# tildearrow/openwebrx

Hardware: NVIDIA B200
Metric: channel-MS/s (input MS/s x clients) + waterfall FFT frames/s (higher is better)
Workload: dtype f32

## Files before the change

### openwebrx_b200/csrc/selector.cu

```cuda
#include "selector_kernels.cuh"
#include "fastconv.cuh"
#include "ingress.cuh"

#include <algorithm>
#include <chrono>
#include <cmath>
#include <complex>
#include <cstdlib>
#include <deque>
#include <map>
#include <memory>
#include <mutex>
#include <vector>

using namespace owrx;

namespace {

int filter_len(double transition)
{
    int len = (int)(4.0 / transition);
    if ((len & 1) == 0) len += 1;
    return len;
}
// ... 248 lines not shown
    float* d_fc_h = nullptr; float2* d_fc_tab = nullptr; float4* d_fc_F = nullptr; float2* d_fc_Z = nullptr;
    float fc_tab_scale = 1.0f;
    float* d_fc_scale = nullptr;
    int* d_fc_slots = nullptr; double* d_fc_rates = nullptr;
    size_t fc_blocks_cap = 0;
    std::vector<double> fc_tab_rate;
    void* d_fc_tabp = nullptr; void* d_fc_Fp = nullptr; size_t fc_blocks_cap_tc = 0;
    std::vector<double> fc_tabp_rate;
    std::vector<float> fc_taps;
};

}

struct owrx_bank {
    int device = 0, sm_count = 0;
    double input_rate = 0.0;
    cudaStream_t stream = nullptr;
    cudaEvent_t ev0 = nullptr, ev1 = nullptr;
    std::mutex mu;
    std::vector<std::unique_ptr<Chan>> chans;
    std::vector<std::unique_ptr<Group>> groups;
    int out_mask = OWRX_OUT_AUDIO;
    float2* d_iq[2] = {nullptr, nullptr};
    int iq_cur = 0;
    size_t iq_cap = 0, iq_fill = 0;
    float* h_stage = nullptr; size_t h_stage_cap = 0;
    float* d_xpose = nullptr; size_t d_xpose_cap = 0;
    struct AsyncDrainItem { int which, width; size_t n, off; std::vector<int> chans; };
    float* h_adrain = nullptr; size_t h_adrain_cap = 0;
    float* d_adrain = nullptr; size_t d_adrain_cap = 0;
    std::vector<AsyncDrainItem> adrain_items;
    bool adrain_pending = false;
    cudaEvent_t adrain_done = nullptr;
    owrx_bank_stats_t stats{};
    cudaStream_t copy_stream = nullptr, side_stream = nullptr, serial_stream = nullptr;
    std::vector<cudaEvent_t> chunk_events;
    cudaEvent_t fir_done = nullptr, ptail_done[2] = {nullptr, nullptr}, tail_done[2] = {nullptr, nullptr}, dev_done = nullptr;
    bool pipelined = false, reserve_sm = false;
    std::vector<cudaEvent_t> fir_events, drain_events;
    cudaStream_t drain_stream = nullptr;
    unsigned long long calls = 0;
    bool profile = false;
    std::vector<std::pair<cudaEvent_t, cudaEvent_t>> prof_events;
    std::vector<int> prof_tags;
    size_t prof_used = 0;
    double prof_ms[OWRX_PROF_KINDS] = {};
    uint64_t prof_launches[OWRX_PROF_KINDS] = {};
    int fir_mode = OWRX_FIR_AUTO, bp_mode = OWRX_FIR_AUTO;
    unsigned char* d_raw = nullptr; size_t raw_cap = 0;
    bool deferred = false, pending_final = false;
    cudaEvent_t carry_done = nullptr;
    int fir_form_used = 0;
    bool tail_fused = true;
    bool agc_cta = true;
    size_t last_consumed = 0;
    std::vector<std::pair<std::unique_ptr<Group>, cudaEvent_t>> graveyard;
    cudaStream_t ctl_stream = nullptr;
    unsigned long long feeds = 0;
};

namespace {

template <typename T> int dev_alloc(T** p, size_t n)
{
    *p = nullptr;
    OWRX_CUDA(cudaMalloc((void**)p, std::max<size_t>(n, 1) * sizeof(T)));
    OWRX_CUDA(cudaMemset(*p, 0, std::max<size_t>(n, 1) * sizeof(T)));
    return OWRX_OK;
}

void group_release(Group* g)
{
    cudaFree(g->d_taps); cudaFree(g->d_deemph); cudaFree(g->d_pre);
    cudaFree(g->d_rate); cudaFree(g->d_phase); cudaFree(g->d_w);
    cudaFree(g->d_bp); cudaFree(g->d_bp_en2[0]); cudaFree(g->d_bp_en2[1]); cudaFree(g->d_cfg2[0]); cudaFree(g->d_cfg2[1]);
    cudaFree(g->d_state); cudaFree(g->d_stash); cudaFree(g->d_patch[0]); cudaFree(g->d_patch[1]);
    cudaFree(g->d_bp_stage); cudaFree(g->d_bp_stage_slots);
    for (int k = 0; k < 2; k++) {
        if (g->h_bp_pin[k]) cudaFreeHost(g->h_bp_pin[k]);
        if (g->bp_pin_ev[k]) cudaEventDestroy(g->bp_pin_ev[k]);
    }
    cudaFree(g->d_bp_H); cudaFree(g->d_bp_X); cudaFree(g->d_bp_Y);
    cudaFree(g->d_partial); cudaFree(g->d_gate); cudaFree(g->d_power); cudaFree(g->d_dcmean); cudaFree(g->d_dcprev);
    cudaFree(g->d_tail_mode2[0]); cudaFree(g->d_tail_mode2[1]); cudaFree(g->d_tail); cudaFree(g->d_tail_count); cudaFree(g->d_tail_s16);
    cudaFree(g->d_tail_bytes);
    cudaFree(g->d_fc_h); cudaFree(g->d_fc_tab); cudaFree(g->d_fc_F); cudaFree(g->d_fc_Z); cudaFree(g->d_fc_slots); cudaFree(g->d_fc_rates);
    cudaFree(g->d_fc_scale);
    cudaFree(g->d_fc_tabp); cudaFree(g->d_fc_Fp);
    g->s1.release(); g->s2.release(); g->s3.release(); g->f1.release(); g->f1p.release(); g->f1b.release(); g->f2.release(); g->f3.release();
}

owrx_chan_spec_t spec_from_rates(double input_rate, double output_rate)
{
    owrx_chan_spec_t sp{};
    double orate = output_rate > input_rate ? input_rate : output_rate;
    const double d = input_rate / orate;
    sp.decimation = (int)d;
    sp.fraction = (input_rate / sp.decimation) / orate;
    sp.transition = 0.15 * (orate / input_rate);
    sp.cutoff = 0.5 * sp.decimation / (input_rate / orate);
    sp.bp_transition = 320.0 / orate;
    sp.squelch_length = std::max(1, (int)(orate / 16));
    sp.deemph_rate = (int)orate;
    return sp;
}

bool spec_equal(const owrx_chan_spec_t& a, const owrx_chan_spec_t& b)
// ... 758 lines not shown
                for (size_t o = 0; o < nv; o += kRowChunk * BP_RB) {
                    const size_t c = std::min(kRowChunk * BP_RB, nv - o);
                    fir_fwd_f_kernel<<<grid2d(S, (c + BP_RB - 1) / BP_RB), kBlock2d, 0, st>>>(src + o * S, S, (int)c, last_row - (int)o, g->d_pre,
                                                                                           g->Tpre, g->f1p.append_ptr() + o * S);
                    OWRX_LAUNCH_CHECK();
                }
                g->f1p.appended(nv);
            }
            size_t cnt = 0;
            while (true) {
                const double where = 5.0 + (double)(g->wfm_m + (long long)cnt) * g->wfm_rate;
                if ((long long)ceil(where) + 6 >= g->f1p.abs_end) break;
                cnt++;
            }
            if ((rc = g->f1b.ensure_new(cnt, st)) != OWRX_OK) return rc;
            if ((rc = g->f2.ensure_new(cnt, st)) != OWRX_OK) return rc;
            for (size_t o = 0; o < cnt; o += kRowChunk) {
                const size_t c = std::min(kRowChunk, cnt - o);
                fracdec_f_kernel<<<grid2d(S, c), kBlock2d, 0, st>>>(g->f1p.rows(), g->f1p.abs_end - (long long)g->f1p.fill, S,
                                                                    g->wfm_rate, g->wfm_m + (long long)o, (int)c, nullptr, 0,
                                                                    g->f1b.append_ptr() + o * S);
                OWRX_LAUNCH_CHECK();
            }
            if (cnt) {
                wfm_deemph_kernel<<<S / IIR_CH, IIR_TL, 0, st>>>(g->f1b.append_ptr(), S, (int)cnt, g->alpha, g->d_state,
                                                                  g->f2.append_ptr());
                OWRX_LAUNCH_CHECK();
            }
            bank->stats.kernel_launches += 2;
            g->wfm_m += (long long)cnt;
            g->f2.appended(cnt);
            n_audio = cnt;
        }
        g->last_demod += n_audio;
        g->last_audio += n_audio;
        g->pass_audio = n_audio;
    }
    return OWRX_OK;
}

int group_tail_serial(owrx_bank* bank, Group* g, cudaStream_t st)
{
    const int S = g->slots;
    const size_t n_audio = g->pass_audio;
    int rc;
    {
        if (n_audio) {
            if ((rc = g->f3.ensure_new(n_audio, st)) != OWRX_OK) return rc;
            if ((rc = prof_mark(bank, OWRX_PROF_AGC, st, true)) != OWRX_OK) return rc;
            if (g->wfm) {
                OWRX_CUDA(cudaMemcpyAsync(g->f3.append_ptr(), g->f2.rows(g->f2.fill - n_audio), n_audio * (size_t)S * sizeof(float),
                                          cudaMemcpyDeviceToDevice, st));
            } else {
                static const int agc_pad = (getenv("OWRX_AGC_PAD_KB") ? atoi(getenv("OWRX_AGC_PAD_KB")) : 160) << 10;
                const bool agc_cta = bank->agc_cta;
                static const int agcw_pad = (getenv("OWRX_AGCW_PAD_KB") ? atoi(getenv("OWRX_AGCW_PAD_KB")) : 0) << 10;
                if (agc_cta) {
                    if (agc_pad) OWRX_CUDA(cudaFuncSetAttribute(agc_kernel, cudaFuncAttributeMaxDynamicSharedMemorySize, agc_pad));
                    agc_kernel<<<S / AGC_CH, AGC_TL, agc_pad, st>>>(g->f2.rows(g->f2.fill - n_audio), S, (int)n_audio, g->d_cfg, g->d_state,
                                                               g->f3.append_ptr());
                } else {
                    if (agcw_pad) OWRX_CUDA(cudaFuncSetAttribute(agc_warp_kernel, cudaFuncAttributeMaxDynamicSharedMemorySize, agcw_pad));
                    agc_warp_kernel<<<S, 32, agcw_pad, st>>>(g->f2.rows(g->f2.fill - n_audio), S, (int)n_audio, g->d_cfg, g->d_state,
                                                           g->f3.append_ptr());
                }
                OWRX_LAUNCH_CHECK();
            }
            if ((rc = prof_mark(bank, OWRX_PROF_AGC, st, false)) != OWRX_OK) return rc;
            bank->stats.kernel_launches++;
            g->f3.appended(n_audio);
            if (g->any_tail) {
                const size_t row0 = g->last_audio - n_audio;
                if (g->last_audio > g->tail_rows_cap) return fail(OWRX_E_STATE, "audio tail scratch under-provisioned");
                audio_tail_kernel<<<(S + 31) / 32, 128, 0, st>>>(g->f3.rows(g->f3.fill - n_audio), S, (int)n_audio, g->d_tail_mode,
                                                               g->d_tail, g->d_tail_s16 + row0 * (size_t)S, g->d_tail_bytes,
                                                               g->d_tail_count, g->tail_cap);
                OWRX_LAUNCH_CHECK();
                bank->stats.kernel_launches++;
                g->tail_ran = true;
            }
        }
    }
    return OWRX_OK;
}

int group_begin_feed(owrx_bank* bank, Group* g, size_t rows, cudaStream_t st_fir, cudaStream_t st_tail, cudaStream_t st_serial, int parity)
{
    const int S = g->slots;
    int rc;
    g->cur = parity & 1;
    const size_t blocks = rows / (size_t)g->sq_len + 2;
    const size_t low = rows + (size_t)g->sq_len + 64;
    if ((rc = g->s1.roll(g->s1.hist, st_fir)) != OWRX_OK) return rc;
    if (g->has_frac && (rc = g->s2.roll(g->s2.hist, st_tail)) != OWRX_OK) return rc;
    if ((rc = g->s3.roll(g->s3.hist, st_tail)) != OWRX_OK) return rc;
    if ((rc = g->f1.roll(g->f1.hist, st_tail)) != OWRX_OK) return rc;
    if (g->wfm) { g->f1b.roll(0, st_tail); if ((rc = g->f1p.roll(g->f1p.hist, st_tail)) != OWRX_OK) return rc; }
    g->f2.roll(0, st_tail);
    g->f3.roll(0, st_tail);
    g->last_audio = g->last_demod = g->last_if = g->last_blocks = 0;
    g->dr_audio = g->dr_demod = g->dr_if = g->dr_blocks = 0;
    g->pass_audio = 0; g->feed_blocks = 0; g->tail_ran = false;
    const bool grow = g->s1.fill + rows > g->s1.cap_rows || (g->has_frac && g->s2.fill + low > g->s2.cap_rows) ||
                      g->s3.fill + low > g->s3.cap_rows || g->f1.fill + low > g->f1.cap_rows || low > g->f2.cap_rows ||
                      low > g->f3.cap_rows || (g->wfm && (low > g->f1b.cap_rows || g->f1p.fill + low > g->f1p.cap_rows)) || blocks > g->blocks_cap ||
                      (g->any_tail && low > g->tail_rows_cap);
    if (grow) {
        OWRX_CUDA(cudaDeviceSynchronize());
        if ((rc = g->s1.ensure_new(rows, st_fir)) != OWRX_OK) return rc;
        if (g->has_frac && (rc = g->s2.ensure_new(low, st_tail)) != OWRX_OK) return rc;
        if ((rc = g->s3.ensure_new(low, st_tail)) != OWRX_OK) return rc;
        if ((rc = g->f1.ensure_new(low, st_tail)) != OWRX_OK) return rc;
        if (g->wfm && (rc = g->f1b.ensure_new(low, st_tail)) != OWRX_OK) return rc;
        if (g->wfm && (rc = g->f1p.ensure_new(low, st_tail)) != OWRX_OK) return rc;
        if ((rc = g->f2.ensure_new(low, st_tail)) != OWRX_OK) return rc;
        if ((rc = g->f3.ensure_new(low, st_tail)) != OWRX_OK) return rc;
        if (blocks > g->blocks_cap) {
// ... 1056 lines not shown
```

### openwebrx_b200/csrc/selector_kernels.cuh

```cuda
#pragma once
#include "common.cuh"
#include "adpcm.cuh"

namespace owrx {

constexpr int K3_NW = 12;
constexpr int K3_CN = 2;
constexpr int K3_PP = 28;
constexpr int K3_RBMAX = 896;
constexpr int K3_CG = 32 * K3_CN;

struct K3Params {
    const float2* iq;
    long long n_lim;
    const float* taps;
    const double* ch_rate;
    const double* ch_phase;
    const float2* ch_w;
    float2* partial;
    float2* side;
    int D, nseg, nrs, RB, JB, n_blocks, n_k, slots;
};

__device__ __forceinline__ void cp_async8(void* smem_dst, const void* gsrc)
// ... 637 lines not shown
            const float4* xv = reinterpret_cast<const float4*>(&xin[buf][w][IIR_E * lane]);
            const float4 a = xv[0], b = xv[1];
            v[0] = a.x; v[1] = a.y; v[2] = a.z; v[3] = a.w; v[4] = b.x; v[5] = b.y; v[6] = b.z; v[7] = b.w;
        }
        float sl = 0.f;
#pragma unroll
        for (int e = 0; e < IIR_E; e++) sl = alpha * v[e] + om * sl;
        float B = sl;
#pragma unroll
        for (int k = 0; k < 5; k++) {
            const float prev = __shfl_up_sync(0xffffffffu, B, 1 << k);
            if (lane >= (1 << k)) B = om_pow[k] * prev + B;
        }
        float A = 1.f;
#pragma unroll
        for (int k = 0; k < 5; k++)
            if ((lane + 1) & (1 << k)) A *= om_pow[k];
        if (lane == 31) A = om_pow[5];
        const float endstate = A * y + B;
        float yin = __shfl_up_sync(0xffffffffu, endstate, 1);
        if (lane == 0) yin = y;
        float yo[IIR_E];
#pragma unroll
        for (int e = 0; e < IIR_E; e++) { yin = alpha * v[e] + om * yin; yo[e] = yin; }
        {
            float4* ov = reinterpret_cast<float4*>(&xout[w][IIR_E * lane]);
            ov[0] = make_float4(yo[0], yo[1], yo[2], yo[3]);
            ov[1] = make_float4(yo[4], yo[5], yo[6], yo[7]);
        }
        const int valid = min(IIR_TL, n - tile * IIR_TL);
        const int ll = (valid - 1) / IIR_E, le = (valid - 1) % IIR_E;
        float cand = yo[IIR_E - 1];
#pragma unroll
        for (int e = 0; e < IIR_E - 1; e++) cand = le == e ? yo[e] : cand;
        y = __shfl_sync(0xffffffffu, cand, ll);
        __syncthreads();
        const int t = tile * IIR_TL + tid;
        if (t < n) {
            float4* p = reinterpret_cast<float4*>(out + (size_t)t * slots + s0);
            p[0] = make_float4(xout[0][tid], xout[1][tid], xout[2][tid], xout[3][tid]);
            p[1] = make_float4(xout[4][tid], xout[5][tid], xout[6][tid], xout[7][tid]);
        }
        if (tile + 1 < nt) stage(buf ^ 1, lo, hi);
        __syncthreads();
    }
    if (lane == 0) st[s].iir = y;
}

constexpr int AGC_CH = 8;
constexpr int AGC_TL = 256;

constexpr int AGC_E = 4;

struct AgcWarp {
    float gain, dn, up, thr, gmax;
    int hang, hang_time;
    __device__ __forceinline__ void step_dense(float (&v)[AGC_E], int lane, float* Ud)
    {
        const unsigned full = 0xffffffffu;
        float o[AGC_E];
        int j0 = 0;
        while (true) {
            const int R = max(32 * AGC_E - j0 - hang, 0);
            float u = gain;
            Ud[3] = u;
#pragma unroll
            for (int c = 0; c < 32 * AGC_E / 4; c++) {
                if (4 * c + 4 <= R) {
                    const float a = u * up, b = a * up, cc = b * up, d = cc * up;
                    *reinterpret_cast<float4*>(&Ud[4 * c + 4]) = make_float4(a, b, cc, d);
                    u = d;
                }
            }
            for (int k = (R & ~3) + 1; k <= R; k++) {
                u *= up;
                Ud[k + 3] = u;
            }
            __syncwarp();
            float gb[AGC_E], ga[AGC_E];
            unsigned att = 0, pend = 0;
#pragma unroll
            for (int e = 0; e < AGC_E; e++) {
                const int d = AGC_E * lane + e - j0;
                const int rb = max(d - hang, 0);
                const int is_rise = d >= hang ? 1 : 0;
                const int idx = max(rb, 0);
                gb[e] = fminf(Ud[idx + 3], gmax);
                ga[e] = fminf(Ud[idx + is_rise + 3], gmax);
                const bool p = d >= 0;
                pend |= (p ? 1u : 0u) << e;
                att |= (p && fabsf(v[e]) * gb[e] > thr ? 1u : 0u) << e;
            }
            __syncwarp();
            const unsigned am = __ballot_sync(full, att != 0u);
            if (am == 0u) {
#pragma unroll
                for (int e = 0; e < AGC_E; e++)
                    if ((pend >> e) & 1u) o[e] = fminf(1.f, fmaxf(-1.f, v[e] * ga[e]));
                gain = fminf(u, gmax);
                hang = max(hang - (32 * AGC_E - j0), 0);
                break;
            }
            const int L = __ffs(am) - 1;
            const int ef = __ffs(att) - 1;
            const float gsel = ef == 0 ? gb[0] : (ef == 1 ? gb[1] : (ef == 2 ? gb[2] : gb[3]));
            const int e_first = __shfl_sync(full, ef, L);
            const float gnew = fmaxf(fminf(__shfl_sync(full, gsel, L) * dn, gmax), 0.f);
            const int jf = AGC_E * L + e_first;
#pragma unroll
            for (int e = 0; e < AGC_E; e++) {
                const int j = AGC_E * lane + e;
                if (((pend >> e) & 1u) && j < jf) o[e] = fminf(1.f, fmaxf(-1.f, v[e] * ga[e]));
                if (j == jf) o[e] = fminf(1.f, fmaxf(-1.f, v[e] * gnew));
            }
            gain = gnew;
            hang = hang_time;
            j0 = jf + 1;
            if (j0 >= 32 * AGC_E) break;
        }
#pragma unroll
        for (int e = 0; e < AGC_E; e++) v[e] = o[e];
    }

    __device__ __forceinline__ void step(float (&v)[AGC_E], int lane, volatile float* U)
    {
        const unsigned full = 0xffffffffu, lt = (1u << lane) - 1u;
        unsigned nzbits = 0;
#pragma unroll
        for (int e = 0; e < AGC_E; e++) nzbits |= (v[e] != 0.f ? 1u : 0u) << e;
        if (__all_sync(full, nzbits == 0xfu)) {
            step_dense(v, lane, const_cast<float*>(U));
            return;
        }
        float o[AGC_E];
#pragma unroll
        for (int e = 0; e < AGC_E; e++) o[e] = v[e];
        int j0 = 0;
        while (true) {
            const int sh = min(max(j0 - AGC_E * lane, 0), AGC_E);
            const unsigned act = (0xfu << sh) & 0xfu;
            const unsigned live = nzbits & act;
            unsigned m[AGC_E];
#pragma unroll
            for (int e = 0; e < AGC_E; e++) m[e] = __ballot_sync(full, (live >> e) & 1u);
            int base = 0, n_live = 0;
#pragma unroll
            for (int e = 0; e < AGC_E; e++) { base += __popc(m[e] & lt); n_live += __popc(m[e]); }
            unsigned rise = 0;
#pragma unroll
            for (int e = 0; e < AGC_E; e++) {
                const int before = base + __popc(live & ((1u << e) - 1u));
                rise |= (((live >> e) & 1u) && before >= hang ? 1u : 0u) << e;
            }
            int rbase = 0, R = 0;
#pragma unroll
            for (int e = 0; e < AGC_E; e++) {
                const unsigned r = __ballot_sync(full, (rise >> e) & 1u);
                rbase += __popc(r & lt);
                R += __popc(r);
            }
            float u = gain;
            U[0] = u;
#pragma unroll 8
            for (int k = 1; k <= R; k++) {
                u *= up;
                U[k] = u;
            }
            __syncwarp();
            float gb[AGC_E], ga[AGC_E];
            unsigned att = 0;
#pragma unroll
            for (int e = 0; e < AGC_E; e++) {
                const int rb = rbase + __popc(rise & ((1u << e) - 1u));
                gb[e] = fminf(U[rb], gmax);
                ga[e] = fminf(U[rb + ((rise >> e) & 1u)], gmax);
                att |= (((live >> e) & 1u) && fabsf(v[e]) * gb[e] > thr ? 1u : 0u) << e;
            }
            __syncwarp();
            const unsigned am = __ballot_sync(full, att != 0u);
            if (am == 0u) {
#pragma unroll
                for (int e = 0; e < AGC_E; e++)
                    if ((act >> e) & 1u) o[e] = fminf(1.f, fmaxf(-1.f, v[e] * ga[e]));
                gain = fminf(u, gmax);
                hang = max(hang - n_live, 0);
                break;
            }
            const int L = __ffs(am) - 1;
            const int ef = __ffs(att) - 1;
            const float gsel = ef == 0 ? gb[0] : (ef == 1 ? gb[1] : (ef == 2 ? gb[2] : gb[3]));
            const int e_first = __shfl_sync(full, ef, L);
            const float gnew = fmaxf(fminf(__shfl_sync(full, gsel, L) * dn, gmax), 0.f);
            const int jf = AGC_E * L + e_first;
#pragma unroll
            for (int e = 0; e < AGC_E; e++) {
                const int j = AGC_E * lane + e;
                if (((act >> e) & 1u) && j < jf) o[e] = fminf(1.f, fmaxf(-1.f, v[e] * ga[e]));
                if (j == jf) o[e] = fminf(1.f, fmaxf(-1.f, v[e] * gnew));
            }
            gain = gnew;
            hang = hang_time;
            j0 = jf + 1;
            if (j0 >= 32 * AGC_E) break;
        }
#pragma unroll
        for (int e = 0; e < AGC_E; e++) v[e] = o[e];
    }
};

__global__ void __launch_bounds__(AGC_TL)
agc_kernel(const float* __restrict__ in, int slots, int n, const ChanCfg* __restrict__ cfg, ChanState* __restrict__ st,
           float* __restrict__ out)
{
    __shared__ __align__(16) float xin[2][AGC_CH][AGC_TL];
    __shared__ __align__(16) float xout[AGC_CH][AGC_TL];
    __shared__ __align__(16) float U_all[AGC_CH][32 * AGC_E + 8];
    if (n <= 0) return;
    const int tid = threadIdx.x, lane = tid & 31, w = tid >> 5;
    const int s0 = blockIdx.x * AGC_CH, s = s0 + w;
    const ChanCfg c = cfg[s];
    const bool bypass = c.kind == OWRX_DEMOD_WFM || c.kind == OWRX_DEMOD_NONE;
    AgcWarp a{st[s].agc_gain, 1.f - c.agc_attack, 1.f + c.agc_decay, c.agc_thr, c.agc_max, st[s].agc_hang, c.agc_hang_time};
    a.gain = fmaxf(fminf(a.gain, a.gmax), 0.f);
    volatile float* U = U_all[w];
    const int nt = (n + AGC_TL - 1) / AGC_TL;
    const float4 zero4 = make_float4(0.f, 0.f, 0.f, 0.f);
    auto fetch = [&](int tile, float4& lo, float4& hi) {
        const int t = tile * AGC_TL + tid;
        if (t < n) {
            const float4* p = reinterpret_cast<const float4*>(in + (size_t)t * slots + s0);
            lo = __ldg(p); hi = __ldg(p + 1);
        } else {
            lo = zero4; hi = zero4;
        }
    };
    auto stage = [&](int buf, const float4& lo, const float4& hi) {
        xin[buf][0][tid] = lo.x; xin[buf][1][tid] = lo.y; xin[buf][2][tid] = lo.z; xin[buf][3][tid] = lo.w;
        xin[buf][4][tid] = hi.x; xin[buf][5][tid] = hi.y; xin[buf][6][tid] = hi.z; xin[buf][7][tid] = hi.w;
    };
    float4 lo, hi;
    fetch(0, lo, hi);
    stage(0, lo, hi);
    __syncthreads();
    for (int tile = 0; tile < nt; tile++) {
        const int buf = tile & 1;
        if (tile + 1 < nt) fetch(tile + 1, lo, hi);
#pragma unroll 1
        for (int k = 0; k < AGC_TL / (32 * AGC_E); k++) {
            const float4 x4 = *reinterpret_cast<const float4*>(&xin[buf][w][k * 32 * AGC_E + AGC_E * lane]);
            float v[AGC_E] = {x4.x, x4.y, x4.z, x4.w};
            if (!bypass) a.step(v, lane, U);
            *reinterpret_cast<float4*>(&xout[w][k * 32 * AGC_E + AGC_E * lane]) = make_float4(v[0], v[1], v[2], v[3]);
        }
        __syncthreads();
        const int t = tile * AGC_TL + tid;
        if (t < n) {
            float4* p = reinterpret_cast<float4*>(out + (size_t)t * slots + s0);
            p[0] = make_float4(xout[0][tid], xout[1][tid], xout[2][tid], xout[3][tid]);
            p[1] = make_float4(xout[4][tid], xout[5][tid], xout[6][tid], xout[7][tid]);
        }
        if (tile + 1 < nt) stage(buf ^ 1, lo, hi);
        __syncthreads();
    }
    if (lane == 0 && !bypass) {
        st[s].agc_gain = a.gain;
        st[s].agc_hang = a.hang;
    }
}

constexpr int AGCW_STAGES = 4;
__global__ void __launch_bounds__(32)
agc_warp_kernel(const float* __restrict__ in, int slots, int n, const ChanCfg* __restrict__ cfg, ChanState* __restrict__ st,
                float* __restrict__ out)
{
    __shared__ __align__(16) float ring[AGCW_STAGES][32 * AGC_E];
    __shared__ __align__(16) float U[32 * AGC_E + 8];
    if (n <= 0) return;
    const int lane = threadIdx.x;
    const int s = blockIdx.x;
    const ChanCfg c = cfg[s];
    const bool bypass = c.kind == OWRX_DEMOD_WFM || c.kind == OWRX_DEMOD_NONE;
    AgcWarp a{st[s].agc_gain, 1.f - c.agc_attack, 1.f + c.agc_decay, c.agc_thr, c.agc_max, st[s].agc_hang, c.agc_hang_time};
    a.gain = fmaxf(fminf(a.gain, a.gmax), 0.f);
    constexpr int SL = 32 * AGC_E;
    const int ns = (n + SL - 1) / SL;
    const float* src = in + s;
    auto issue = [&](int step) {
        if (step < ns) {
            const int i0 = step * SL + AGC_E * lane;
#pragma unroll
            for (int e = 0; e < AGC_E; e++) {
                float* dst = &ring[step % AGCW_STAGES][AGC_E * lane + e];
                if (i0 + e < n) cp_async4(dst, src + (size_t)(i0 + e) * slots);
                else *dst = 0.f;
            }
        }
        cp_async_commit();
    };
#pragma unroll
    for (int k = 0; k < AGCW_STAGES - 1; k++) issue(k);
    for (int step = 0; step < ns; step++) {
        issue(step + AGCW_STAGES - 1);
        cp_async_wait<AGCW_STAGES - 1>();
        __syncwarp();
        const float4 x4 = *reinterpret_cast<const float4*>(&ring[step % AGCW_STAGES][AGC_E * lane]);
        float v[AGC_E] = {x4.x, x4.y, x4.z, x4.w};
        if (!bypass) a.step(v, lane, U);
        const int i0 = step * SL + AGC_E * lane;
#pragma unroll
        for (int e = 0; e < AGC_E; e++)
            if (i0 + e < n) out[(size_t)(i0 + e) * slots + s] = v[e];
        __syncwarp();
    }
    if (lane == 0 && !bypass) {
        st[s].agc_gain = a.gain;
        st[s].agc_hang = a.hang;
    }
}

template <typename T>
__global__ void __launch_bounds__(256) transpose_kernel(const T* __restrict__ in, int slots, size_t n, T* __restrict__ out)
{
    __shared__ T tile[32][33];
    const int s0 = blockIdx.x * 32;
    const size_t i0 = (size_t)blockIdx.y * 32;
    for (int r = threadIdx.y; r < 32; r += 8) {
        const size_t i = i0 + r;
        const int sl = s0 + threadIdx.x;
        if (i < n && sl < slots) tile[r][threadIdx.x] = in[i * slots + sl];
    }
    __syncthreads();
    for (int r = threadIdx.y; r < 32; r += 8) {
        const int sl = s0 + r;
        const size_t i = i0 + threadIdx.x;
        if (i < n && sl < slots) out[(size_t)sl * n + i] = tile[threadIdx.x][r];
    }
}

struct TailState {
    int index, pred, since_sync, have_lo, lo;
};

constexpr int AT_R = 32;
constexpr int AT_OB = 36;
__device__ __forceinline__ void at_bar_sync(int id) { asm volatile("barrier.sync %0, 128;" ::"r"(id) : "memory"); }
__device__ __forceinline__ void at_bar_arrive(int id) { asm volatile("barrier.arrive %0, 128;" ::"r"(id) : "memory"); }

__global__ void __launch_bounds__(128)
audio_tail_kernel(const float* __restrict__ in, int slots, int n, const int* __restrict__ mode, TailState* __restrict__ ts,
                  int16_t* __restrict__ s16_out, unsigned char* __restrict__ bytes_out, int* __restrict__ count_out, int cap)
{
    __shared__ uint4 succ[IMA_TABLE_ENTRIES];
    __shared__ int qt[2][AT_R][32];
    __shared__ unsigned char obuf[2][32][AT_OB];
    __shared__ int onb[2][32];
    const int lane = threadIdx.x & 31, w = threadIdx.x >> 5;
    ima_build_table(succ, threadIdx.x, 128);
    const int s = blockIdx.x * 32 + lane;
    const bool live = s < slots;
    const int sc = live ? s : slots - 1;
    const int md = live ? mode[sc] : 0;
    if (__syncthreads_and(md == 0)) return;
    const int n_tiles = (n + AT_R - 1) / AT_R;
    constexpr int FULL = 1, EMPTY = 3;
    if (w == 0) {
// ... 137 lines not shown
```

Measured before the change: 3.549 million.

## Replace per-channel warp AGC with 512-sample tiled multi-channel AGC kernel

Replaces the one-warp-per-channel cp.async AGC kernel with a tile kernel in which each block handles 8 channels. Each warp processes 512 samples (16 per lane) per step, and loads and stores go through a shared-memory transpose using coalesced float4 accesses. AgcWarp becomes a template over elements per lane. The dense path now fills the gain ramp in chunks of 16 and stops early once the gain hits its maximum, skipping the ramp entirely when already saturated. The default switches to this new path, with dynamic shared memory padded to the device opt-in maximum to limit occupancy. The risks are more register pressure from 16 values per lane and serialized warps when attacks are frequent.

```diff
diff --git a/openwebrx_b200/csrc/selector.cu b/openwebrx_b200/csrc/selector.cu
--- a/openwebrx_b200/csrc/selector.cu
+++ b/openwebrx_b200/csrc/selector.cu
@@ -324,7 +324,7 @@
     cudaEvent_t carry_done = nullptr;
     int fir_form_used = 0;
     bool tail_fused = true;
-    bool agc_cta = true;
+    bool agc_cta = false;
     size_t last_consumed = 0;
     std::vector<std::pair<std::unique_ptr<Group>, cudaEvent_t>> graveyard;
     cudaStream_t ctl_stream = nullptr;
@@ -1189,17 +1189,26 @@
                 OWRX_CUDA(cudaMemcpyAsync(g->f3.append_ptr(), g->f2.rows(g->f2.fill - n_audio), n_audio * (size_t)S * sizeof(float),
                                           cudaMemcpyDeviceToDevice, st));
             } else {
-                static const int agc_pad = (getenv("OWRX_AGC_PAD_KB") ? atoi(getenv("OWRX_AGC_PAD_KB")) : 160) << 10;
-                const bool agc_cta = bank->agc_cta;
-                static const int agcw_pad = (getenv("OWRX_AGCW_PAD_KB") ? atoi(getenv("OWRX_AGCW_PAD_KB")) : 0) << 10;
-                if (agc_cta) {
+                static const int pad_env = getenv("OWRX_AGC_PAD_KB") ? atoi(getenv("OWRX_AGC_PAD_KB")) << 10 : -1;
+                if (bank->agc_cta) {
+                    const int agc_pad = pad_env >= 0 ? pad_env : 160 << 10;
                     if (agc_pad) OWRX_CUDA(cudaFuncSetAttribute(agc_kernel, cudaFuncAttributeMaxDynamicSharedMemorySize, agc_pad));
                     agc_kernel<<<S / AGC_CH, AGC_TL, agc_pad, st>>>(g->f2.rows(g->f2.fill - n_audio), S, (int)n_audio, g->d_cfg, g->d_state,
                                                                g->f3.append_ptr());
                 } else {
-                    if (agcw_pad) OWRX_CUDA(cudaFuncSetAttribute(agc_warp_kernel, cudaFuncAttributeMaxDynamicSharedMemorySize, agcw_pad));
-                    agc_warp_kernel<<<S, 32, agcw_pad, st>>>(g->f2.rows(g->f2.fill - n_audio), S, (int)n_audio, g->d_cfg, g->d_state,
-                                                           g->f3.append_ptr());
+                    static int full_pad = -1;
+                    if (full_pad < 0) {
+                        int dev = 0, optin = 0;
+                        cudaFuncAttributes fa{};
+                        OWRX_CUDA(cudaGetDevice(&dev));
+                        OWRX_CUDA(cudaDeviceGetAttribute(&optin, cudaDevAttrMaxSharedMemoryPerBlockOptin, dev));
+                        OWRX_CUDA(cudaFuncGetAttributes(&fa, agc_tile_kernel));
+                        full_pad = std::max(optin - (int)fa.sharedSizeBytes, 0);
+                    }
+                    const int agc_pad = pad_env >= 0 ? pad_env : full_pad;
+                    if (agc_pad) OWRX_CUDA(cudaFuncSetAttribute(agc_tile_kernel, cudaFuncAttributeMaxDynamicSharedMemorySize, agc_pad));
+                    agc_tile_kernel<<<S / AGC_CH, AGC_TL, agc_pad, st>>>(g->f2.rows(g->f2.fill - n_audio), S, (int)n_audio, g->d_cfg,
+                                                                    g->d_state, g->f3.append_ptr());
                 }
                 OWRX_LAUNCH_CHECK();
             }
diff --git a/openwebrx_b200/csrc/selector_kernels.cuh b/openwebrx_b200/csrc/selector_kernels.cuh
--- a/openwebrx_b200/csrc/selector_kernels.cuh
+++ b/openwebrx_b200/csrc/selector_kernels.cuh
@@ -713,109 +713,125 @@
 
 constexpr int AGC_E = 4;
 
+template <int E>
 struct AgcWarp {
+    static constexpr int W = 32 * E;
     float gain, dn, up, thr, gmax;
     int hang, hang_time;
-    __device__ __forceinline__ void step_dense(float (&v)[AGC_E], int lane, float* Ud)
+    __device__ __forceinline__ void step_dense(float (&v)[E], int lane, float* Ud)
     {
         const unsigned full = 0xffffffffu;
-        float o[AGC_E];
+        float o[E];
         int j0 = 0;
         while (true) {
-            const int R = max(32 * AGC_E - j0 - hang, 0);
+            const int R = max(W - j0 - hang, 0);
             float u = gain;
-            Ud[3] = u;
-#pragma unroll
-            for (int c = 0; c < 32 * AGC_E / 4; c++) {
-                if (4 * c + 4 <= R) {
-                    const float a = u * up, b = a * up, cc = b * up, d = cc * up;
-                    *reinterpret_cast<float4*>(&Ud[4 * c + 4]) = make_float4(a, b, cc, d);
-                    u = d;
+            int kv = 0;
+            float gu[E + 1];
+            if (R > 0 && u < gmax) {
+                Ud[3] = u;
+                kv = R;
+                int k = 0;
+                for (; k + 16 <= R; k += 16) {
+                    float t[16];
+                    t[0] = u * up;
+#pragma unroll
+                    for (int i = 1; i < 16; i++) t[i] = t[i - 1] * up;
+#pragma unroll
+                    for (int q = 0; q < 4; q++)
+                        *reinterpret_cast<float4*>(&Ud[k + 4 + 4 * q]) = make_float4(t[4 * q], t[4 * q + 1], t[4 * q + 2], t[4 * q + 3]);
+                    u = t[15];
+                    if (u >= gmax) { kv = k + 16; k = R; break; }
                 }
-            }
-            for (int k = (R & ~3) + 1; k <= R; k++) {
-                u *= up;
-                Ud[k + 3] = u;
-            }
-            __syncwarp();
-            float gb[AGC_E], ga[AGC_E];
-            unsigned att = 0, pend = 0;
-#pragma unroll
-            for (int e = 0; e < AGC_E; e++) {
-                const int d = AGC_E * lane + e - j0;
-                const int rb = max(d - hang, 0);
-                const int is_rise = d >= hang ? 1 : 0;
-                const int idx = max(rb, 0);
-                gb[e] = fminf(Ud[idx + 3], gmax);
-                ga[e] = fminf(Ud[idx + is_rise + 3], gmax);
-                const bool p = d >= 0;
-                pend |= (p ? 1u : 0u) << e;
-                att |= (p && fabsf(v[e]) * gb[e] > thr ? 1u : 0u) << e;
-            }
-            __syncwarp();
+#pragma unroll
+                for (int i = 0; i < 15; i++)
+                    if (k + i < R) {
+                        u *= up;
+                        Ud[k + 4 + i] = u;
+                    }
+                __syncwarp();
+#pragma unroll
+                for (int e = 0; e <= E; e++) {
+                    const int idx = max(E * lane + e - j0 - hang, 0);
+                    gu[e] = idx <= kv ? fminf(Ud[idx + 3], gmax) : gmax;
+                }
+                __syncwarp();
+            } else {
+#pragma unroll
+                for (int e = 0; e <= E; e++) gu[e] = gain;
+            }
+            unsigned att = 0;
+#pragma unroll
+            for (int e = 0; e < E; e++) {
+                const bool p = E * lane + e >= j0;
+                att |= (p && fabsf(v[e]) * gu[e] > thr ? 1u : 0u) << e;
+            }
             const unsigned am = __ballot_sync(full, att != 0u);
             if (am == 0u) {
 #pragma unroll
-                for (int e = 0; e < AGC_E; e++)
-                    if ((pend >> e) & 1u) o[e] = fminf(1.f, fmaxf(-1.f, v[e] * ga[e]));
+                for (int e = 0; e < E; e++)
+                    if (E * lane + e >= j0) o[e] = fminf(1.f, fmaxf(-1.f, v[e] * gu[e + 1]));
                 gain = fminf(u, gmax);
-                hang = max(hang - (32 * AGC_E - j0), 0);
+                hang = max(hang - (W - j0), 0);
                 break;
             }
             const int L = __ffs(am) - 1;
             const int ef = __ffs(att) - 1;
-            const float gsel = ef == 0 ? gb[0] : (ef == 1 ? gb[1] : (ef == 2 ? gb[2] : gb[3]));
+            float gsel = gu[0];
+#pragma unroll
+            for (int e = 1; e < E; e++) if (ef == e) gsel = gu[e];
             const int e_first = __shfl_sync(full, ef, L);
             const float gnew = fmaxf(fminf(__shfl_sync(full, gsel, L) * dn, gmax), 0.f);
-            const int jf = AGC_E * L + e_first;
-#pragma unroll
-            for (int e = 0; e < AGC_E; e++) {
-                const int j = AGC_E * lane + e;
-                if (((pend >> e) & 1u) && j < jf) o[e] = fminf(1.f, fmaxf(-1.f, v[e] * ga[e]));
+            const int jf = E * L + e_first;
+#pragma unroll
+            for (int e = 0; e < E; e++) {
+                const int j = E * lane + e;
+                if (j >= j0 && j < jf) o[e] = fminf(1.f, fmaxf(-1.f, v[e] * gu[e + 1]));
                 if (j == jf) o[e] = fminf(1.f, fmaxf(-1.f, v[e] * gnew));
             }
             gain = gnew;
             hang = hang_time;
             j0 = jf + 1;
-            if (j0 >= 32 * AGC_E) break;
-        }
-#pragma unroll
-        for (int e = 0; e < AGC_E; e++) v[e] = o[e];
-    }
-
-    __device__ __forceinline__ void step(float (&v)[AGC_E], int lane, volatile float* U)
+            if (j0 >= W) break;
+        }
+#pragma unroll
+        for (int e = 0; e < E; e++) v[e] = o[e];
+    }
+
+    __device__ __forceinline__ void step(float (&v)[E], int lane, volatile float* U)
     {
         const unsigned full = 0xffffffffu, lt = (1u << lane) - 1u;
+        constexpr unsigned all = (1u << E) - 1u;
         unsigned nzbits = 0;
 #pragma unroll
-        for (int e = 0; e < AGC_E; e++) nzbits |= (v[e] != 0.f ? 1u : 0u) << e;
-        if (__all_sync(full, nzbits == 0xfu)) {
+        for (int e = 0; e < E; e++) nzbits |= (v[e] != 0.f ? 1u : 0u) << e;
+        if (__all_sync(full, nzbits == all)) {
             step_dense(v, lane, const_cast<float*>(U));
             return;
         }
-        float o[AGC_E];
-#pragma unroll
-        for (int e = 0; e < AGC_E; e++) o[e] = v[e];
+        float o[E];
+#pragma unroll
+        for (int e = 0; e < E; e++) o[e] = v[e];
         int j0 = 0;
         while (true) {
-            const int sh = min(max(j0 - AGC_E * lane, 0), AGC_E);
-            const unsigned act = (0xfu << sh) & 0xfu;
+            const int sh = min(max(j0 - E * lane, 0), E);
+            const unsigned act = (all << sh) & all;
             const unsigned live = nzbits & act;
-            unsigned m[AGC_E];
-#pragma unroll
-            for (int e = 0; e < AGC_E; e++) m[e] = __ballot_sync(full, (live >> e) & 1u);
+            unsigned m[E];
+#pragma unroll
+            for (int e = 0; e < E; e++) m[e] = __ballot_sync(full, (live >> e) & 1u);
             int base = 0, n_live = 0;
 #pragma unroll
-            for (int e = 0; e < AGC_E; e++) { base += __popc(m[e] & lt); n_live += __popc(m[e]); }
+            for (int e = 0; e < E; e++) { base += __popc(m[e] & lt); n_live += __popc(m[e]); }
             unsigned rise = 0;
 #pragma unroll
-            for (int e = 0; e < AGC_E; e++) {
+            for (int e = 0; e < E; e++) {
                 const int before = base + __popc(live & ((1u << e) - 1u));
                 rise |= (((live >> e) & 1u) && before >= hang ? 1u : 0u) << e;
             }
             int rbase = 0, R = 0;
 #pragma unroll
-            for (int e = 0; e < AGC_E; e++) {
+            for (int e = 0; e < E; e++) {
                 const unsigned r = __ballot_sync(full, (rise >> e) & 1u);
                 rbase += __popc(r & lt);
                 R += __popc(r);
@@ -828,10 +844,10 @@
                 U[k] = u;
             }
             __syncwarp();
-            float gb[AGC_E], ga[AGC_E];
+            float gb[E], ga[E];
             unsigned att = 0;
 #pragma unroll
-            for (int e = 0; e < AGC_E; e++) {
+            for (int e = 0; e < E; e++) {
                 const int rb = rbase + __popc(rise & ((1u << e) - 1u));
                 gb[e] = fminf(U[rb], gmax);
                 ga[e] = fminf(U[rb + ((rise >> e) & 1u)], gmax);
@@ -841,7 +857,7 @@
             const unsigned am = __ballot_sync(full, att != 0u);
             if (am == 0u) {
 #pragma unroll
-                for (int e = 0; e < AGC_E; e++)
+                for (int e = 0; e < E; e++)
                     if ((act >> e) & 1u) o[e] = fminf(1.f, fmaxf(-1.f, v[e] * ga[e]));
                 gain = fminf(u, gmax);
                 hang = max(hang - n_live, 0);
@@ -849,23 +865,25 @@
             }
             const int L = __ffs(am) - 1;
             const int ef = __ffs(att) - 1;
-            const float gsel = ef == 0 ? gb[0] : (ef == 1 ? gb[1] : (ef == 2 ? gb[2] : gb[3]));
+            float gsel = gb[0];
+#pragma unroll
+            for (int e = 1; e < E; e++) if (ef == e) gsel = gb[e];
             const int e_first = __shfl_sync(full, ef, L);
             const float gnew = fmaxf(fminf(__shfl_sync(full, gsel, L) * dn, gmax), 0.f);
-            const int jf = AGC_E * L + e_first;
-#pragma unroll
-            for (int e = 0; e < AGC_E; e++) {
-                const int j = AGC_E * lane + e;
+            const int jf = E * L + e_first;
+#pragma unroll
+            for (int e = 0; e < E; e++) {
+                const int j = E * lane + e;
                 if (((act >> e) & 1u) && j < jf) o[e] = fminf(1.f, fmaxf(-1.f, v[e] * ga[e]));
                 if (j == jf) o[e] = fminf(1.f, fmaxf(-1.f, v[e] * gnew));
             }
             gain = gnew;
             hang = hang_time;
             j0 = jf + 1;
-            if (j0 >= 32 * AGC_E) break;
-        }
-#pragma unroll
-        for (int e = 0; e < AGC_E; e++) v[e] = o[e];
+            if (j0 >= W) break;
+        }
+#pragma unroll
+        for (int e = 0; e < E; e++) v[e] = o[e];
     }
 };
 
@@ -881,7 +899,7 @@
     const int s0 = blockIdx.x * AGC_CH, s = s0 + w;
     const ChanCfg c = cfg[s];
     const bool bypass = c.kind == OWRX_DEMOD_WFM || c.kind == OWRX_DEMOD_NONE;
-    AgcWarp a{st[s].agc_gain, 1.f - c.agc_attack, 1.f + c.agc_decay, c.agc_thr, c.agc_max, st[s].agc_hang, c.agc_hang_time};
+    AgcWarp<AGC_E> a{st[s].agc_gain, 1.f - c.agc_attack, 1.f + c.agc_decay, c.agc_thr, c.agc_max, st[s].agc_hang, c.agc_hang_time};
     a.gain = fmaxf(fminf(a.gain, a.gmax), 0.f);
     volatile float* U = U_all[w];
     const int nt = (n + AGC_TL - 1) / AGC_TL;
@@ -929,49 +947,68 @@
     }
 }
 
-constexpr int AGCW_STAGES = 4;
-__global__ void __launch_bounds__(32)
-agc_warp_kernel(const float* __restrict__ in, int slots, int n, const ChanCfg* __restrict__ cfg, ChanState* __restrict__ st,
+constexpr int AGCT_E = 16;
+constexpr int AGCT_TL = 32 * AGCT_E;
+constexpr int AGCT_LD = AGCT_TL + 4;
+__global__ void __launch_bounds__(AGC_TL)
+agc_tile_kernel(const float* __restrict__ in, int slots, int n, const ChanCfg* __restrict__ cfg, ChanState* __restrict__ st,
                 float* __restrict__ out)
 {
-    __shared__ __align__(16) float ring[AGCW_STAGES][32 * AGC_E];
-    __shared__ __align__(16) float U[32 * AGC_E + 8];
+    __shared__ __align__(16) float x[AGC_CH][AGCT_LD];
+    __shared__ __align__(16) float U_all[AGC_CH][AGCT_TL + 8];
     if (n <= 0) return;
-    const int lane = threadIdx.x;
-    const int s = blockIdx.x;
+    const int tid = threadIdx.x, lane = tid & 31, w = tid >> 5;
+    const int s0 = blockIdx.x * AGC_CH, s = s0 + w;
     const ChanCfg c = cfg[s];
     const bool bypass = c.kind == OWRX_DEMOD_WFM || c.kind == OWRX_DEMOD_NONE;
-    AgcWarp a{st[s].agc_gain, 1.f - c.agc_attack, 1.f + c.agc_decay, c.agc_thr, c.agc_max, st[s].agc_hang, c.agc_hang_time};
+    AgcWarp<AGCT_E> a{st[s].agc_gain, 1.f - c.agc_attack, 1.f + c.agc_decay, c.agc_thr, c.agc_max, st[s].agc_hang, c.agc_hang_time};
     a.gain = fmaxf(fminf(a.gain, a.gmax), 0.f);
-    constexpr int SL = 32 * AGC_E;
-    const int ns = (n + SL - 1) / SL;
-    const float* src = in + s;
-    auto issue = [&](int step) {
-        if (step < ns) {
-            const int i0 = step * SL + AGC_E * lane;
-#pragma unroll
-            for (int e = 0; e < AGC_E; e++) {
-                float* dst = &ring[step % AGCW_STAGES][AGC_E * lane + e];
-                if (i0 + e < n) cp_async4(dst, src + (size_t)(i0 + e) * slots);
-                else *dst = 0.f;
-            }
-        }
-        cp_async_commit();
+    float* U = U_all[w];
+    const int nt = (n + AGCT_TL - 1) / AGCT_TL;
+    constexpr int RPI = AGC_TL / 2;
+    constexpr int NP = AGCT_TL / RPI;
+    const int h = tid & 1, r0 = tid >> 1;
+    float4 pre[NP];
+    auto fetch = [&](int tile) {
+#pragma unroll
+        for (int p = 0; p < NP; p++) {
+            const int t = tile * AGCT_TL + p * RPI + r0;
+            pre[p] = t < n ? __ldg(reinterpret_cast<const float4*>(in + (size_t)t * slots + s0) + h)
+                           : make_float4(0.f, 0.f, 0.f, 0.f);
+        }
     };
-#pragma unroll
-    for (int k = 0; k < AGCW_STAGES - 1; k++) issue(k);
-    for (int step = 0; step < ns; step++) {
-        issue(step + AGCW_STAGES - 1);
-        cp_async_wait<AGCW_STAGES - 1>();
-        __syncwarp();
-        const float4 x4 = *reinterpret_cast<const float4*>(&ring[step % AGCW_STAGES][AGC_E * lane]);
-        float v[AGC_E] = {x4.x, x4.y, x4.z, x4.w};
+    auto stage = [&]() {
+#pragma unroll
+        for (int p = 0; p < NP; p++) {
+            const int r = p * RPI + r0;
+            x[4 * h][r] = pre[p].x; x[4 * h + 1][r] = pre[p].y; x[4 * h + 2][r] = pre[p].z; x[4 * h + 3][r] = pre[p].w;
+        }
+    };
+    fetch(0);
+    stage();
+    __syncthreads();
+    for (int tile = 0; tile < nt; tile++) {
+        if (tile + 1 < nt) fetch(tile + 1);
+        float v[AGCT_E];
+#pragma unroll
+        for (int q = 0; q < AGCT_E / 4; q++) {
+            const float4 x4 = *reinterpret_cast<const float4*>(&x[w][AGCT_E * lane + 4 * q]);
+            v[4 * q] = x4.x; v[4 * q + 1] = x4.y; v[4 * q + 2] = x4.z; v[4 * q + 3] = x4.w;
+        }
         if (!bypass) a.step(v, lane, U);
-        const int i0 = step * SL + AGC_E * lane;
-#pragma unroll
-        for (int e = 0; e < AGC_E; e++)
-            if (i0 + e < n) out[(size_t)(i0 + e) * slots + s] = v[e];
-        __syncwarp();
+#pragma unroll
+        for (int q = 0; q < AGCT_E / 4; q++)
+            *reinterpret_cast<float4*>(&x[w][AGCT_E * lane + 4 * q]) = make_float4(v[4 * q], v[4 * q + 1], v[4 * q + 2], v[4 * q + 3]);
+        __syncthreads();
+#pragma unroll
+        for (int p = 0; p < NP; p++) {
+            const int r = p * RPI + r0, t = tile * AGCT_TL + r;
+            if (t < n)
+                reinterpret_cast<float4*>(out + (size_t)t * slots + s0)[h] =
+                    make_float4(x[4 * h][r], x[4 * h + 1][r], x[4 * h + 2][r], x[4 * h + 3][r]);
+        }
+        if (tile + 1 < nt) stage();
+        __syncthreads();
     }
     if (lane == 0 && !bypass) {
         st[s].agc_gain = a.gain;
```

Measured after the change: 3.587 million (median of 6 runs). 1.1% higher.

## Replace warp-per-channel AGC with pipelined CTA kernel and software-pipelined gain chain

Applied to the files above, without the earlier changes.

Replaces the single-warp-per-channel AGC kernel with a 256-thread kernel that handles 8 channels per block. It stages 1024-sample tiles through double-buffered dynamic shared memory, using coalesced float4 loads and stores, and makes this the default path instead of the previous CTA kernel. The AGC step now precomputes the next step's gain-ramp chain while processing the current one, and skips chain computation when gain is flat (saturated, zero, or in hang). This is meant to shorten the serial per-sample recurrence and improve memory coalescing. The cost is more shared memory per block (the padded size plus 20 KB), which may lower occupancy, and more complex control flow.

```diff
diff --git a/openwebrx_b200/csrc/selector.cu b/openwebrx_b200/csrc/selector.cu
--- a/openwebrx_b200/csrc/selector.cu
+++ b/openwebrx_b200/csrc/selector.cu
@@ -324,7 +324,7 @@
     cudaEvent_t carry_done = nullptr;
     int fir_form_used = 0;
     bool tail_fused = true;
-    bool agc_cta = true;
+    bool agc_cta = false;
     size_t last_consumed = 0;
     std::vector<std::pair<std::unique_ptr<Group>, cudaEvent_t>> graveyard;
     cudaStream_t ctl_stream = nullptr;
@@ -1190,16 +1190,14 @@
                                           cudaMemcpyDeviceToDevice, st));
             } else {
                 static const int agc_pad = (getenv("OWRX_AGC_PAD_KB") ? atoi(getenv("OWRX_AGC_PAD_KB")) : 160) << 10;
-                const bool agc_cta = bank->agc_cta;
-                static const int agcw_pad = (getenv("OWRX_AGCW_PAD_KB") ? atoi(getenv("OWRX_AGCW_PAD_KB")) : 0) << 10;
-                if (agc_cta) {
+                const float* f2 = g->f2.rows(g->f2.fill - n_audio);
+                if (bank->agc_cta) {
                     if (agc_pad) OWRX_CUDA(cudaFuncSetAttribute(agc_kernel, cudaFuncAttributeMaxDynamicSharedMemorySize, agc_pad));
-                    agc_kernel<<<S / AGC_CH, AGC_TL, agc_pad, st>>>(g->f2.rows(g->f2.fill - n_audio), S, (int)n_audio, g->d_cfg, g->d_state,
-                                                               g->f3.append_ptr());
+                    agc_kernel<<<S / AGC_CH, AGC_TL, agc_pad, st>>>(f2, S, (int)n_audio, g->d_cfg, g->d_state, g->f3.append_ptr());
                 } else {
-                    if (agcw_pad) OWRX_CUDA(cudaFuncSetAttribute(agc_warp_kernel, cudaFuncAttributeMaxDynamicSharedMemorySize, agcw_pad));
-                    agc_warp_kernel<<<S, 32, agcw_pad, st>>>(g->f2.rows(g->f2.fill - n_audio), S, (int)n_audio, g->d_cfg, g->d_state,
-                                                           g->f3.append_ptr());
+                    const int smem = std::max(AGCP_SMEM, agc_pad ? agc_pad + (20 << 10) : 0);
+                    OWRX_CUDA(cudaFuncSetAttribute(agc_pipe_kernel, cudaFuncAttributeMaxDynamicSharedMemorySize, smem));
+                    agc_pipe_kernel<<<S / AGC_CH, AGC_TL, smem, st>>>(f2, S, (int)n_audio, g->d_cfg, g->d_state, g->f3.append_ptr());
                 }
                 OWRX_LAUNCH_CHECK();
             }
diff --git a/openwebrx_b200/csrc/selector_kernels.cuh b/openwebrx_b200/csrc/selector_kernels.cuh
--- a/openwebrx_b200/csrc/selector_kernels.cuh
+++ b/openwebrx_b200/csrc/selector_kernels.cuh
@@ -718,9 +718,15 @@
     int hang, hang_time;
     __device__ __forceinline__ void step_dense(float (&v)[AGC_E], int lane, float* Ud)
     {
+        float o[AGC_E];
+        dense_from(v, o, lane, Ud, 0);
+#pragma unroll
+        for (int e = 0; e < AGC_E; e++) v[e] = o[e];
+    }
+
+    __device__ __forceinline__ void dense_from(const float (&v)[AGC_E], float (&o)[AGC_E], int lane, float* Ud, int j0)
+    {
         const unsigned full = 0xffffffffu;
-        float o[AGC_E];
-        int j0 = 0;
         while (true) {
             const int R = max(32 * AGC_E - j0 - hang, 0);
             float u = gain;
@@ -779,20 +785,23 @@
             j0 = jf + 1;
             if (j0 >= 32 * AGC_E) break;
         }
-#pragma unroll
-        for (int e = 0; e < AGC_E; e++) v[e] = o[e];
     }
 
     __device__ __forceinline__ void step(float (&v)[AGC_E], int lane, volatile float* U)
     {
-        const unsigned full = 0xffffffffu, lt = (1u << lane) - 1u;
         unsigned nzbits = 0;
 #pragma unroll
         for (int e = 0; e < AGC_E; e++) nzbits |= (v[e] != 0.f ? 1u : 0u) << e;
-        if (__all_sync(full, nzbits == 0xfu)) {
+        if (__all_sync(0xffffffffu, nzbits == 0xfu)) {
             step_dense(v, lane, const_cast<float*>(U));
             return;
         }
+        step_sparse(v, lane, U, nzbits);
+    }
+
+    __device__ __forceinline__ void step_sparse(float (&v)[AGC_E], int lane, volatile float* U, unsigned nzbits)
+    {
+        const unsigned full = 0xffffffffu, lt = (1u << lane) - 1u;
         float o[AGC_E];
 #pragma unroll
         for (int e = 0; e < AGC_E; e++) o[e] = v[e];
@@ -866,6 +875,89 @@
         }
 #pragma unroll
         for (int e = 0; e < AGC_E; e++) v[e] = o[e];
+    }
+
+    __device__ __forceinline__ bool flat(float g, int h) const { return (g == gmax && up >= 1.f) || g == 0.f || h >= 32 * AGC_E; }
+
+    __device__ __forceinline__ void chain(float u, float* Ud) const
+    {
+        Ud[3] = u;
+#pragma unroll
+        for (int c = 0; c < 32 * AGC_E / 4; c++) {
+            const float a = u * up, b = a * up, cc = b * up, d = cc * up;
+            *reinterpret_cast<float4*>(&Ud[4 * c + 4]) = make_float4(a, b, cc, d);
+            u = d;
+        }
+    }
+
+    template <bool NEXT>
+    __device__ __forceinline__ unsigned pass0(const float (&v)[AGC_E], int lane, const float* Uc, bool cst, float gn, float* Un,
+                                              float (&gb)[AGC_E], float (&o)[AGC_E], unsigned& att) const
+    {
+        float ga[AGC_E];
+#pragma unroll
+        for (int e = 0; e < AGC_E; e++) {
+            const int d = AGC_E * lane + e;
+            const int rb = max(d - hang, 0);
+            const int is_rise = d >= hang ? 1 : 0;
+            gb[e] = cst ? gain : fminf(Uc[rb + 3], gmax);
+            ga[e] = cst ? gain : fminf(Uc[rb + is_rise + 3], gmax);
+        }
+        if (NEXT) chain(gn, Un);
+        att = 0;
+#pragma unroll
+        for (int e = 0; e < AGC_E; e++) {
+            att |= (fabsf(v[e]) * gb[e] > thr ? 1u : 0u) << e;
+            o[e] = fminf(1.f, fmaxf(-1.f, v[e] * ga[e]));
+        }
+        return __ballot_sync(0xffffffffu, att != 0u);
+    }
+
+    __device__ __forceinline__ bool step_pipe(float (&v)[AGC_E], int lane, float* Uc, float* Un, bool ready)
+    {
+        const unsigned full = 0xffffffffu;
+        unsigned nzbits = 0;
+#pragma unroll
+        for (int e = 0; e < AGC_E; e++) nzbits |= (v[e] != 0.f ? 1u : 0u) << e;
+        __syncwarp();
+        if (!__all_sync(full, nzbits == 0xfu)) {
+            step_sparse(v, lane, Uc, nzbits);
+            return false;
+        }
+        const bool cst = flat(gain, hang);
+        if (!cst && !ready) {
+            chain(gain, Uc);
+            __syncwarp();
+        }
+        const int hn = max(hang - 32 * AGC_E, 0);
+        const float gn = cst ? gain : fminf(Uc[max(32 * AGC_E - hang, 0) + 3], gmax);
+        float gb[AGC_E], o[AGC_E];
+        unsigned att;
+        const unsigned am = flat(gn, hn) ? pass0<false>(v, lane, Uc, cst, gn, Un, gb, o, att)
+                                         : pass0<true>(v, lane, Uc, cst, gn, Un, gb, o, att);
+        if (am == 0u) {
+            gain = gn;
+            hang = hn;
+#pragma unroll
+            for (int e = 0; e < AGC_E; e++) v[e] = o[e];
+            return true;
+        }
+        const int L = __ffs(am) - 1;
+        const int ef = __ffs(att) - 1;
+        const float gsel = ef == 0 ? gb[0] : (ef == 1 ? gb[1] : (ef == 2 ? gb[2] : gb[3]));
+        const int e_first = __shfl_sync(full, ef, L);
+        const float gnew = fmaxf(fminf(__shfl_sync(full, gsel, L) * dn, gmax), 0.f);
+        const int jf = AGC_E * L + e_first;
+#pragma unroll
+        for (int e = 0; e < AGC_E; e++)
+            if (AGC_E * lane + e == jf) o[e] = fminf(1.f, fmaxf(-1.f, v[e] * gnew));
+        gain = gnew;
+        hang = hang_time;
+        __syncwarp();
+        if (jf + 1 < 32 * AGC_E) dense_from(v, o, lane, Uc, jf + 1);
+#pragma unroll
+        for (int e = 0; e < AGC_E; e++) v[e] = o[e];
+        return false;
     }
 };
 
@@ -929,49 +1021,76 @@
     }
 }
 
-constexpr int AGCW_STAGES = 4;
-__global__ void __launch_bounds__(32)
-agc_warp_kernel(const float* __restrict__ in, int slots, int n, const ChanCfg* __restrict__ cfg, ChanState* __restrict__ st,
+constexpr int AGCP_TL = 1024;
+constexpr int AGCP_ROWS = AGCP_TL / AGC_TL;
+constexpr int AGCP_SMEM = 2 * AGC_CH * AGCP_TL * (int)sizeof(float);
+__global__ void __launch_bounds__(AGC_TL)
+agc_pipe_kernel(const float* __restrict__ in, int slots, int n, const ChanCfg* __restrict__ cfg, ChanState* __restrict__ st,
                 float* __restrict__ out)
 {
-    __shared__ __align__(16) float ring[AGCW_STAGES][32 * AGC_E];
-    __shared__ __align__(16) float U[32 * AGC_E + 8];
+    constexpr int SL = 32 * AGC_E;
+    extern __shared__ __align__(16) float agcp_dyn[];
+    float (*xin)[AGC_CH][AGCP_TL] = reinterpret_cast<float (*)[AGC_CH][AGCP_TL]>(agcp_dyn);
+    __shared__ __align__(16) float Ub[AGC_CH][2][SL + 8];
     if (n <= 0) return;
-    const int lane = threadIdx.x;
-    const int s = blockIdx.x;
+    const int tid = threadIdx.x, lane = tid & 31, w = tid >> 5;
+    const int s0 = blockIdx.x * AGC_CH, s = s0 + w;
     const ChanCfg c = cfg[s];
     const bool bypass = c.kind == OWRX_DEMOD_WFM || c.kind == OWRX_DEMOD_NONE;
     AgcWarp a{st[s].agc_gain, 1.f - c.agc_attack, 1.f + c.agc_decay, c.agc_thr, c.agc_max, st[s].agc_hang, c.agc_hang_time};
     a.gain = fmaxf(fminf(a.gain, a.gmax), 0.f);
-    constexpr int SL = 32 * AGC_E;
-    const int ns = (n + SL - 1) / SL;
-    const float* src = in + s;
-    auto issue = [&](int step) {
-        if (step < ns) {
-            const int i0 = step * SL + AGC_E * lane;
-#pragma unroll
-            for (int e = 0; e < AGC_E; e++) {
-                float* dst = &ring[step % AGCW_STAGES][AGC_E * lane + e];
-                if (i0 + e < n) cp_async4(dst, src + (size_t)(i0 + e) * slots);
-                else *dst = 0.f;
-            }
-        }
-        cp_async_commit();
+    const int nt = (n + AGCP_TL - 1) / AGCP_TL;
+    const float4 zero4 = make_float4(0.f, 0.f, 0.f, 0.f);
+    float4 lo[AGCP_ROWS], hi[AGCP_ROWS];
+    auto fetch = [&](int tile) {
+#pragma unroll
+        for (int r = 0; r < AGCP_ROWS; r++) {
+            const int t = tile * AGCP_TL + r * AGC_TL + tid;
+            if (t < n) {
+                const float4* p = reinterpret_cast<const float4*>(in + (size_t)t * slots + s0);
+                lo[r] = __ldg(p); hi[r] = __ldg(p + 1);
+            } else {
+                lo[r] = zero4; hi[r] = zero4;
+            }
+        }
     };
-#pragma unroll
-    for (int k = 0; k < AGCW_STAGES - 1; k++) issue(k);
-    for (int step = 0; step < ns; step++) {
-        issue(step + AGCW_STAGES - 1);
-        cp_async_wait<AGCW_STAGES - 1>();
-        __syncwarp();
-        const float4 x4 = *reinterpret_cast<const float4*>(&ring[step % AGCW_STAGES][AGC_E * lane]);
-        float v[AGC_E] = {x4.x, x4.y, x4.z, x4.w};
-        if (!bypass) a.step(v, lane, U);
-        const int i0 = step * SL + AGC_E * lane;
-#pragma unroll
-        for (int e = 0; e < AGC_E; e++)
-            if (i0 + e < n) out[(size_t)(i0 + e) * slots + s] = v[e];
-        __syncwarp();
+    auto stage = [&](int buf) {
+#pragma unroll
+        for (int r = 0; r < AGCP_ROWS; r++) {
+            const int i = r * AGC_TL + tid;
+            xin[buf][0][i] = lo[r].x; xin[buf][1][i] = lo[r].y; xin[buf][2][i] = lo[r].z; xin[buf][3][i] = lo[r].w;
+            xin[buf][4][i] = hi[r].x; xin[buf][5][i] = hi[r].y; xin[buf][6][i] = hi[r].z; xin[buf][7][i] = hi[r].w;
+        }
+    };
+    fetch(0);
+    stage(0);
+    __syncthreads();
+    bool ready = false;
+    int k = 0;
+    for (int tile = 0; tile < nt; tile++) {
+        const int buf = tile & 1;
+        if (tile + 1 < nt) fetch(tile + 1);
+        const int steps = min(AGCP_TL / SL, (n - tile * AGCP_TL + SL - 1) / SL);
+#pragma unroll 1
+        for (int j = 0; j < steps; j++, k++) {
+            float4* x = reinterpret_cast<float4*>(&xin[buf][w][j * SL + AGC_E * lane]);
+            const float4 x4 = *x;
+            float v[AGC_E] = {x4.x, x4.y, x4.z, x4.w};
+            if (!bypass) ready = a.step_pipe(v, lane, Ub[w][k & 1], Ub[w][(k + 1) & 1], ready);
+            *x = make_float4(v[0], v[1], v[2], v[3]);
+        }
+        __syncthreads();
+#pragma unroll
+        for (int r = 0; r < AGCP_ROWS; r++) {
+            const int i = r * AGC_TL + tid, t = tile * AGCP_TL + i;
+            if (t < n) {
+                float4* p = reinterpret_cast<float4*>(out + (size_t)t * slots + s0);
+                p[0] = make_float4(xin[buf][0][i], xin[buf][1][i], xin[buf][2][i], xin[buf][3][i]);
+                p[1] = make_float4(xin[buf][4][i], xin[buf][5][i], xin[buf][6][i], xin[buf][7][i]);
+            }
+        }
+        if (tile + 1 < nt) stage(buf ^ 1);
+        __syncthreads();
     }
     if (lane == 0 && !bypass) {
         st[s].agc_gain = a.gain;
```

Result: faster. 3.552 million before, 3.596 million after (median of 6 runs) (+1.2%).
